# shionhonda/IaGo

Hardware: AMD Instinct MI355X
Metric: self-play games/sec (higher is better)
Workload: dtype f16 MFMA operands (float32 split in 2 / 3 pieces), f32 accumulate; u64 bitboards; f32 / f64 tree statistics

## Files before the change

### iago_amd/csrc/conv_policy_body.hpp

```cpp
#pragma once
#include "abi_common.hpp"

#include <hip/hip_fp16.h>

#include <cstdlib>

#include <atomic>

namespace iago_policy {


typedef _Float16 half8 __attribute__((ext_vector_type(8)));
typedef float float16v __attribute__((ext_vector_type(16)));
typedef float float4v __attribute__((ext_vector_type(4)));
#define IAGO_POLICY_MFMA16(acc, a, b) asm volatile("v_mfma_f32_16x16x32_f16 %0, %1, %2, %0" : "+a"(acc) : "v"(a), "v"(b))
typedef unsigned int u32x4 __attribute__((ext_vector_type(4)));
typedef float f2 __attribute__((ext_vector_type(2)));
typedef _Float16 h2 __attribute__((ext_vector_type(2)));

constexpr int RS = 800;
constexpr int ZB = 1280;
constexpr int BS = 64 * RS + ZB;
constexpr int HEAD_FLOATS = 64;
constexpr int W1_LDS = (64 * 18 + 64) * 4;
constexpr int LDS_BYTES = BS + 1024 + HEAD_FLOATS * 4 + W1_LDS;
constexpr float S1 = 1.0f / 2048.0f, S2 = 1.0f / (2048.0f * 2048.0f);

struct PolicyParams {
    const uint64_t *own, *opp;
    const int64_t *index;
    const int32_t *n_dev;
    int64_t n;
    const float *w1, *b1;
    const uint4 *w_hi[7], *w_mid[7], *w_lo[7];
    const float *bias[7];
    const float *w9, *b10;
    float *probs;
    uint32_t *overflow;
    int layer_lo, layer_hi;
    uint4 *scratch;
    int64_t row_lo, row_hi;
};

__device__ __forceinline__ void split3(const f2 v, h2 &hi, h2 &mid, h2 &lo)
{
    hi = __builtin_convertvector(v, h2);
    const f2 r1 = (v - __builtin_convertvector(hi, f2)) * 2048.0f;
    mid = __builtin_convertvector(r1, h2);
    const f2 r2 = (r1 - __builtin_convertvector(mid, f2)) * 2048.0f;
    lo = __builtin_convertvector(r2, h2);
}

extern __shared__ __align__(16) char policy_lds[];

template <bool SRCH = false>
__device__ __forceinline__ void policy_item(const PolicyParams &P, const int64_t row_id, const uint32_t *pos = nullptr,
                                            float *res = nullptr, const float *w1_staged = nullptr,
                                            const float *head_w = nullptr)
{
    char *const T = policy_lds;
    int tid_ = threadIdx.x;
    if constexpr (SRCH)
        asm volatile("" : "+v"(tid_));
    const int tid = tid_, wv = __builtin_amdgcn_readfirstlane(tid >> 6), lane = tid & 63;
    const int64_t b = P.index ? P.index[row_id] : row_id;

    if (tid < ZB / 16)
        *(uint4 *)(T + 64 * RS + tid * 16) = make_uint4(0, 0, 0, 0);
    bool saturated = false;
    if (P.layer_lo > 0) {
        const uint4 *src = P.scratch + (row_id - P.row_lo) * (64 * RS / 16);
        for (int e = tid; e < 64 * RS / 16; e += 256)
            *(uint4 *)(T + e * 16) = src[e];
    } else {
        const int cell = tid & 63, y = cell >> 3, x = cell & 7;
        const uint64_t bits0 = SRCH ? (((uint64_t)pos[5] << 32) | pos[4]) : P.opp[b];
        const uint64_t bits1 = SRCH ? (((uint64_t)pos[3] << 32) | pos[2]) : P.own[b];
        float in[18];
#pragma unroll
        for (int c = 0; c < 2; c++)
#pragma unroll
            for (int ky = 0; ky < 3; ky++)
#pragma unroll
                for (int kx = 0; kx < 3; kx++) {
                    const int yy = y + ky - 1, xx = x + kx - 1;
                    const bool ok = yy >= 0 && yy < 8 && xx >= 0 && xx < 8;
                    const int a = (yy * 8 + xx) & 63;
                    in[c * 9 + ky * 3 + kx] = (ok && (((c ? bits1 : bits0) >> a) & 1ull)) ? 1.0f : 0.0f;
                }
        const float *w1s = w1_staged;
        if constexpr (!SRCH) {
            float *const st = (float *)(T + BS + 1024 + HEAD_FLOATS * 4);
            for (int e = tid; e < 64 * 18 / 4; e += 256)
                ((float4 *)st)[e] = ((const float4 *)P.w1)[e];
            if (tid < 16)
                ((float4 *)(st + 64 * 18))[tid] = ((const float4 *)P.b1)[tid];
            __syncthreads();
            w1s = st;
        }
#pragma unroll 1
        for (int g2 = 0; g2 < 2; g2++) {
            const int grp = __builtin_amdgcn_readfirstlane(g2 * 4 + wv);
            const int co0 = grp * 8;
            _Float16 p0[8], p1[8], p2[8];
#pragma unroll
            for (int k = 0; k < 8; k += 2) {
                const float *wa = w1s + (co0 + k) * 18, *wb = wa + 18;
                f2 acc = (f2){w1s[64 * 18 + co0 + k], w1s[64 * 18 + co0 + k + 1]};
#pragma unroll
                for (int j = 0; j < 18; j++)
                    acc = __builtin_elementwise_fma((f2){wa[j], wb[j]}, (f2){in[j], in[j]}, acc);
                saturated |= !(acc.x <= 65000.0f) || !(acc.y <= 65000.0f);
                f2 v;
                v.x = fminf(fmaxf(acc.x, 0.0f), 65000.0f);
                v.y = fminf(fmaxf(acc.y, 0.0f), 65000.0f);
                h2 a0, a1, a2;
                split3(v, a0, a1, a2);
                p0[k] = a0.x, p0[k + 1] = a0.y;
                p1[k] = a1.x, p1[k + 1] = a1.y;
                p2[k] = a2.x, p2[k + 1] = a2.y;
            }
            char *dst = T + cell * RS + (grp >> 1) * 32 + (grp & 1) * 16;
            *(uint4 *)dst = *(const uint4 *)p0;
            *(uint4 *)(dst + 256) = *(const uint4 *)p1;
            *(uint4 *)(dst + 512) = *(const uint4 *)p2;
        }
    }
    __syncthreads();

    const int c16 = lane & 15, kq = lane >> 4;
    uint32_t addr[4][9];
#pragma unroll
    for (int q = 0; q < 4; q++)
#pragma unroll
        for (int tap = 0; tap < 9; tap++) {
            const int cell = 16 * q + c16;
            const int yy = (cell >> 3) + tap / 3 - 1, xx = (cell & 7) + tap % 3 - 1;
            const bool ok = yy >= 0 && yy < 8 && xx >= 0 && xx < 8;
            const int lin = (cell + (tap / 3 - 1) * 8 + (tap % 3 - 1)) & 7;
            addr[q][tap] = (uint32_t)((ok ? (yy * 8 + xx) * RS : 64 * RS + 32 * lin) + kq * 16);
        }
    uint32_t wrow[4];
#pragma unroll
    for (int q = 0; q < 4; q++)
        wrow[q] = (uint32_t)((16 * q + c16) * RS);

    for (int L = P.layer_lo; L < P.layer_hi; L++) {
        const int n_pairs = L == 0 ? 2 : 4;
        const char *const wh = (const char *)P.w_hi[L], *const wm = (const char *)P.w_mid[L], *const wl = (const char *)P.w_lo[L];
        const uint32_t a_lane = (uint32_t)(((32 * wv + c16) * 2 + (kq & 1) + (kq >> 1) * (9 * 256)) * 16);
        auto a_load = [&](const char *base, uint32_t step_bytes, int m) -> u32x4 {
            return *(const u32x4 *)(base + step_bytes + a_lane + (uint32_t)m * 512u);
        };
        float4v acc0[2][4], acc0b[2][4], acc1[2][4], acc2[2][4];
#pragma unroll
        for (int m = 0; m < 2; m++)
#pragma unroll
            for (int n = 0; n < 4; n++)
#pragma unroll
                for (int v = 0; v < 4; v++) {
                    acc0[m][n][v] = 0.0f;
                    acc0b[m][n][v] = 0.0f;
                    acc1[m][n][v] = 0.0f;
                    acc2[m][n][v] = 0.0f;
                }
        u32x4 a_hi[3][2], a_mid[3][2], a_lo[3][2];
#pragma unroll
        for (int i = 0; i < 2; i++)
#pragma unroll
            for (int m = 0; m < 2; m++) {
                a_hi[i][m] = a_load(wh, (uint32_t)i * 4096u, m);
                a_mid[i][m] = a_load(wm, (uint32_t)i * 4096u, m);
                a_lo[i][m] = a_load(wl, (uint32_t)i * 4096u, m);
            }
        half8 bh[3], bm[3], bl[3];
        auto b_addr = [&](int tile) -> const char * {
            const int over = tile >= 36 ? 64 : 0, tt = tile % 36;
            return T + addr[tt & 3][tt >> 2] + over;
        };
        {
            const char *p0 = b_addr(0), *p1 = b_addr(1);
            bh[0] = *(const half8 *)p0, bm[0] = *(const half8 *)(p0 + 256), bl[0] = *(const half8 *)(p0 + 512);
            bh[1] = *(const half8 *)p1, bm[1] = *(const half8 *)(p1 + 256), bl[1] = *(const half8 *)(p1 + 512);
        }
        for (int cp = 0; cp < n_pairs; cp++) {
#pragma unroll
            for (int tap = 0; tap < 9; tap++) {
                int cp2 = cp, tp2 = tap + 2;
                if (tp2 >= 9) {
                    tp2 -= 9;
                    cp2 += 1;
                }
                if (cp2 >= n_pairs) {
                    cp2 = n_pairs - 1;
                    tp2 = 8;
                }
                const uint32_t w2 = (uint32_t)(18 * cp2 + tp2) * 4096u;
                half8 ah[2], am[2], al[2];
#pragma unroll
                for (int m = 0; m < 2; m++) {
                    ah[m] = __builtin_bit_cast(half8, a_hi[tap % 3][m]);
                    am[m] = __builtin_bit_cast(half8, a_mid[tap % 3][m]);
                    al[m] = __builtin_bit_cast(half8, a_lo[tap % 3][m]);
                }
#pragma unroll
                for (int q = 0; q < 4; q++) {
                    const int tile = tap * 4 + q, cur = tile % 3, nxt = (tile + 2) % 3;
                    const char *p = b_addr(tile + 2);
                    __builtin_amdgcn_sched_barrier(0);
                    IAGO_POLICY_MFMA16(acc2[0][q], ah[0], bl[cur]);
                    bh[nxt] = *(const half8 *)p;
                    __builtin_amdgcn_sched_barrier(0);
                    IAGO_POLICY_MFMA16(acc2[1][q], ah[1], bl[cur]);
                    bm[nxt] = *(const half8 *)(p + 256);
                    __builtin_amdgcn_sched_barrier(0);
                    IAGO_POLICY_MFMA16(acc1[0][q], ah[0], bm[cur]);
                    bl[nxt] = *(const half8 *)(p + 512);
                    __builtin_amdgcn_sched_barrier(0);
                    IAGO_POLICY_MFMA16(acc1[1][q], ah[1], bm[cur]);
                    if (q == 0)
                        a_hi[(tap + 2) % 3][0] = a_load(wh, w2, 0);
                    else if (q == 1)
                        a_mid[(tap + 2) % 3][0] = a_load(wm, w2, 0);
                    else if (q == 2)
                        a_lo[(tap + 2) % 3][0] = a_load(wl, w2, 0);
                    __builtin_amdgcn_sched_barrier(0);
                    if (tap & 1)
                        IAGO_POLICY_MFMA16(acc0b[0][q], ah[0], bh[cur]);
                    else
                        IAGO_POLICY_MFMA16(acc0[0][q], ah[0], bh[cur]);
                    if (q == 0)
                        a_hi[(tap + 2) % 3][1] = a_load(wh, w2, 1);
                    else if (q == 1)
                        a_mid[(tap + 2) % 3][1] = a_load(wm, w2, 1);
                    else if (q == 2)
                        a_lo[(tap + 2) % 3][1] = a_load(wl, w2, 1);
                    __builtin_amdgcn_sched_barrier(0);
                    if (tap & 1)
                        IAGO_POLICY_MFMA16(acc0b[1][q], ah[1], bh[cur]);
                    else
                        IAGO_POLICY_MFMA16(acc0[1][q], ah[1], bh[cur]);
                    IAGO_POLICY_MFMA16(acc2[0][q], al[0], bh[cur]);
                    IAGO_POLICY_MFMA16(acc2[1][q], al[1], bh[cur]);
                    IAGO_POLICY_MFMA16(acc1[0][q], am[0], bh[cur]);
                    IAGO_POLICY_MFMA16(acc1[1][q], am[1], bh[cur]);
                    IAGO_POLICY_MFMA16(acc2[0][q], am[0], bm[cur]);
                    IAGO_POLICY_MFMA16(acc2[1][q], am[1], bm[cur]);
                    __builtin_amdgcn_sched_barrier(0);
                }
            }
#pragma unroll
            for (int q = 0; q < 4; q++)
#pragma unroll
                for (int tap = 0; tap < 9; tap++)
                    addr[q][tap] += 64u;
        }
#pragma unroll
        for (int q = 0; q < 4; q++)
#pragma unroll
            for (int tap = 0; tap < 9; tap++)
                addr[q][tap] -= 64u * (uint32_t)n_pairs;

        f2 bia[2][2];
#pragma unroll
        for (int m = 0; m < 2; m++) {
            const float4 bq = *(const float4 *)(P.bias[L] + 32 * wv + 16 * m + 4 * kq);
            bia[m][0] = (f2){bq.x, bq.y};
            bia[m][1] = (f2){bq.z, bq.w};
        }
        asm volatile("s_nop 15\n\ts_nop 7" ::: "memory");
        __syncthreads();
        float vmax = 0.0f;
        f2 vsum = (f2){0.0f, 0.0f};
#pragma unroll
        for (int q = 0; q < 4; q++) {
            char *row = T + wrow[q] + (32 * wv + 4 * kq) * 2;
#pragma unroll
            for (int m = 0; m < 2; m++) {
                h2 p0[2], p1[2], p2[2];
#pragma unroll
                for (int t2 = 0; t2 < 2; t2++) {
                    const f2 m0 = (f2){acc0[m][q][2 * t2], acc0[m][q][2 * t2 + 1]} + (f2){acc0b[m][q][2 * t2], acc0b[m][q][2 * t2 + 1]};
                    const f2 m1 = (f2){acc1[m][q][2 * t2], acc1[m][q][2 * t2 + 1]};
                    const f2 m2 = (f2){acc2[m][q][2 * t2], acc2[m][q][2 * t2 + 1]};
                    f2 v = (m2 * S2 + m1 * S1) + m0 + bia[m][t2];
                    vmax = fmaxf(fmaxf(vmax, v.x), v.y);
                    vsum += v;
                    v.x = __builtin_amdgcn_fmed3f(v.x, 0.0f, 65000.0f);
                    v.y = __builtin_amdgcn_fmed3f(v.y, 0.0f, 65000.0f);
                    split3(v, p0[t2], p1[t2], p2[t2]);
                }
                *(uint2 *)(row + 32 * m) = (uint2){__builtin_bit_cast(uint32_t, p0[0]), __builtin_bit_cast(uint32_t, p0[1])};
                *(uint2 *)(row + 32 * m + 256) =
                    (uint2){__builtin_bit_cast(uint32_t, p1[0]), __builtin_bit_cast(uint32_t, p1[1])};
                *(uint2 *)(row + 32 * m + 512) =
                    (uint2){__builtin_bit_cast(uint32_t, p2[0]), __builtin_bit_cast(uint32_t, p2[1])};
            }
        }
        saturated |= !(vmax <= 65000.0f) || !(vsum.x + vsum.y == vsum.x + vsum.y);
        __syncthreads();
    }
    if (P.overflow && saturated)
        *P.overflow = 1u;
    if (P.layer_hi < 7) {
        uint4 *dst = P.scratch + (row_id - P.row_lo) * (64 * RS / 16);
        for (int e = tid; e < 64 * RS / 16; e += 256)
            dst[e] = *(const uint4 *)(T + e * 16);
        return;
    }

    if (wv == 0) {
        const char *row = T + lane * RS;
        float acc = 0.0f;
#pragma unroll 4
        for (int c8 = 0; c8 < 16; c8++) {
            const half8 xh = *(const half8 *)(row + c8 * 16), xm = *(const half8 *)(row + 256 + c8 * 16),
                        xl = *(const half8 *)(row + 512 + c8 * 16);
            const float *w9 = SRCH ? head_w : P.w9;
            const float4 wa = *(const float4 *)(w9 + c8 * 8), wb = *(const float4 *)(w9 + c8 * 8 + 4);
            const float w[8] = {wa.x, wa.y, wa.z, wa.w, wb.x, wb.y, wb.z, wb.w};
#pragma unroll
            for (int e = 0; e < 8; e++) {
                const float xv = ((float)xl[e] * S2 + (float)xm[e] * S1) + (float)xh[e];
                acc = fmaf(w[e], xv, acc);
            }
        }
        const float logit = acc + (SRCH ? head_w[128 + lane] : P.b10[lane]);
        float mx = logit;
#pragma unroll
        for (int o = 32; o > 0; o >>= 1)
            mx = fmaxf(mx, __shfl_xor(mx, o));
        const float e = expf(logit - mx);
        float sum = e;
#pragma unroll
        for (int o = 32; o > 0; o >>= 1)
            sum += __shfl_xor(sum, o);
        if constexpr (SRCH)
            res[lane] = e / sum;
        else
            P.probs[row_id * 64 + lane] = e / sum;
    }
}

inline int policy_params_of(const iago_policy_split3_args *a, PolicyParams &P)
{
    if (!a || a->n < 0)
        return iago_fail(IAGO_ERR_INVALID, "iago_policy_forward_split3: null args or n < 0");
    if (!a->own || !a->opp || !a->w1 || !a->b1 || !a->w9 || !a->b10 || !a->probs)
        return iago_fail(IAGO_ERR_INVALID, "iago_policy_forward_split3: null pointer");
    for (int L = 0; L < 7; L++) {
        if (!a->w_hi[L] || !a->w_mid[L] || !a->w_lo[L] || !a->bias[L] || ((uintptr_t)a->w_hi[L] & 15u) ||
            ((uintptr_t)a->w_mid[L] & 15u) || ((uintptr_t)a->w_lo[L] & 15u) || ((uintptr_t)a->bias[L] & 15u))
            return iago_fail(IAGO_ERR_INVALID, "iago_policy_forward_split3: weights and biases of blocks 2..8 must be "
                                               "non-null and 16-byte aligned");
        P.w_hi[L] = (const uint4 *)a->w_hi[L];
        P.w_mid[L] = (const uint4 *)a->w_mid[L];
        P.w_lo[L] = (const uint4 *)a->w_lo[L];
        P.bias[L] = a->bias[L];
    }
    if (((uintptr_t)a->w9 & 15u) || ((uintptr_t)a->w1 & 15u) || ((uintptr_t)a->b1 & 15u))
        return iago_fail(IAGO_ERR_INVALID, "iago_policy_forward_split3: w1, b1, w9 must be 16-byte aligned");
    P.own = a->own;
    P.opp = a->opp;
    P.index = a->index;
    P.n_dev = a->n_dev;
    P.n = a->n;
    P.w1 = a->w1;
    P.b1 = a->b1;
    P.w9 = a->w9;
    P.b10 = a->b10;
    P.probs = a->probs;
    P.overflow = a->overflow;
    P.layer_lo = 0;
    P.layer_hi = 7;
    P.scratch = nullptr;
    P.row_lo = 0;
    P.row_hi = a->n;
    return IAGO_OK;
}

}
```

### iago_amd/csrc/conv_trunk_body.hpp

```cpp
#pragma once
#include "abi_common.hpp"
#include "rollout_row_body.hpp"

#include <hip/hip_fp16.h>

#include <atomic>
#include <type_traits>

namespace iago_trunk {


typedef _Float16 half8 __attribute__((ext_vector_type(8)));
typedef float float16v __attribute__((ext_vector_type(16)));
typedef float float4v __attribute__((ext_vector_type(4)));
typedef unsigned int u32x4 __attribute__((ext_vector_type(4)));
typedef float f2 __attribute__((ext_vector_type(2)));
typedef _Float16 h2 __attribute__((ext_vector_type(2)));

constexpr int RS = 544;
constexpr int ZB = 1024;
constexpr int BS = 64 * RS + ZB;
constexpr int lds_alloc(int tb) { return tb * BS + 1024; }
constexpr int MAX_LAYERS = 8;

#define IAGO_MFMA16(acc, a, b) asm volatile("v_mfma_f32_16x16x32_f16 %0, %1, %2, %0" : "+a"(acc) : "v"(a), "v"(b))

struct TrunkRParams {
    const uint4 *x_hi, *x_lo;
    uint4 *y_hi, *y_lo;
    const uint4 *w_hi[MAX_LAYERS], *w_lo[MAX_LAYERS];
    const float *bias[MAX_LAYERS];
    int64_t n;
    int32_t cin0, n_layers;
    uint32_t *overflow;
    const float *planes;
    const uint64_t *own, *opp;
    const float *w1, *b1;
    const uint4 *w9_hi, *w9_lo;
    const float *b9, *w10, *w11;
    float *out;
    const int64_t *index;
    const int32_t *n_dev;
    int32_t count_lo, count_hi;
    int32_t layer_lo, layer_hi;
    char *scratch;
};
constexpr int IMG = 64 * RS;

struct Piece {
    const int64_t *index;
    const int32_t *n_dev;
    char *scratch;
    int layer_lo, layer_hi;
    const uint32_t *pos;
    float *res;
    const float *w1s;
    const char *head_w;
};
constexpr int HEAD_W_W9LO = 8192, HEAD_W_W10 = 16384, HEAD_W_W11 = 16384 + 32768, HEAD_W_B9 = HEAD_W_W11 + 512,
              HEAD_W_LDS = HEAD_W_B9 + 16;
__device__ __forceinline__ Piece whole_walk(const TrunkRParams &P)
{
    return Piece{P.index, P.n_dev, P.scratch, P.layer_lo, P.layer_hi, nullptr, nullptr, nullptr, nullptr};
}

constexpr int head_lds(int tb) { return (9 * 64 * tb + 64 * tb + 128 * tb) * 4; }
constexpr int W1_LDS = (64 * 18 + 64) * 4;
constexpr int lds_alloc_fused(int tb) { return lds_alloc(tb) + head_lds(tb) + W1_LDS; }

__device__ __forceinline__ int cell_of_lane(int r)
{
    return r < 4 ? r : r < 12 ? 16 + (r - 4) : r < 16 ? 4 + (r - 12) : r < 20 ? 24 + (r - 16) : r < 28 ? 8 + (r - 20)
                                                                                              : 28 + (r - 28);
}

extern __shared__ __align__(16) char trunk_lds[];

constexpr bool tile_off_board(int tb, int tap, int n)
{
    return tb >= 2 && ((tap < 3 && (n & 7) == 0) || (tap >= 6 && (n & 7) == 7));
}
constexpr int kept_before(int tb, int tap, int n)
{
    int k = 0;
    for (int t = 0; t < 9; t++)
        for (int m = 0; m < 4 * tb; m++) {
            if (t == tap && m == n)
                return k;
            k += !tile_off_board(tb, t, m);
        }
    return k;
}
constexpr int kept_tile(int tb, int k)
{
    for (int t = 0; t < 9; t++)
        for (int m = 0; m < 4 * tb; m++)
            if (!tile_off_board(tb, t, m) && k-- == 0)
                return t * 4 * tb + m;
    return -1;
}
template <int I0, int I1, class F>
__device__ __forceinline__ void static_for(F &&f)
{
    if constexpr (I0 < I1) {
        f(std::integral_constant<int, I0>{});
        static_for<I0 + 1, I1>(f);
    }
}

template <bool FUSED, int TB, bool SRCH = false>
__device__ __forceinline__ void trunk_item(const TrunkRParams &P, const Piece &W, const int64_t b0, const int64_t n_rows)
{
    constexpr int NN = 4 * TB;
    char *const T = trunk_lds;
    int tid_ = threadIdx.x;
    if constexpr (SRCH)
        asm volatile("" : "+v"(tid_));
    const int tid = tid_, wv = __builtin_amdgcn_readfirstlane(tid >> 6), lane = tid & 63, r = lane & 31, h = lane >> 5;

    if (tid < TB * (ZB / 16))
        *(uint4 *)(T + (tid / (ZB / 16)) * BS + 64 * RS + (tid % (ZB / 16)) * 16) = make_uint4(0, 0, 0, 0);
    bool saturated = false;
    constexpr bool PIECES = FUSED && TB <= 2;
    if (PIECES && W.layer_lo > 0) {
        constexpr int PER = (TB * (IMG / 16) + 255) / 256;
        uint4 img[PER];
#pragma unroll
        for (int i = 0; i < PER; i++) {
            const int e = min(tid + i * 256, TB * (IMG / 16) - 1);
            const int board = e / (IMG / 16), off = e - board * (IMG / 16);
            const int64_t row = min(b0 + board, n_rows - 1);
            img[i] = ((const uint4 *)(W.scratch + row * IMG))[off];
        }
#pragma unroll
        for (int i = 0; i < PER; i++) {
            const int e = tid + i * 256;
            const int board = e / (IMG / 16), off = e - board * (IMG / 16);
            if (e < TB * (IMG / 16))
                *(uint4 *)(T + board * BS + off * 16) = img[i];
        }
    } else if constexpr (FUSED) {
        const int cell = tid & 63, y = cell >> 3, x = cell & 7;
        float in[TB][18];
#pragma unroll
        for (int board = 0; board < TB; board++) {
            const int64_t row = min(b0 + board, n_rows - 1);
            const int64_t b = W.index ? W.index[row] : row;
            const float *pl = P.planes + b * 128;
            uint64_t bits0, bits1;
            if constexpr (SRCH) {
                const uint32_t *w = W.pos + 6 * board;
                bits1 = ((uint64_t)w[3] << 32) | w[2];
                bits0 = ((uint64_t)w[5] << 32) | w[4];
            } else {
                bits0 = P.planes ? 0ull : P.opp[b];
                bits1 = P.planes ? 0ull : P.own[b];
            }
#pragma unroll
            for (int c = 0; c < 2; c++)
#pragma unroll
                for (int ky = 0; ky < 3; ky++)
#pragma unroll
                    for (int kx = 0; kx < 3; kx++) {
                        const int yy = y + ky - 1, xx = x + kx - 1;
                        const bool ok = yy >= 0 && yy < 8 && xx >= 0 && xx < 8;
                        const int a = (yy * 8 + xx) & 63;
                        float v;
                        if (P.planes)
                            v = ok ? pl[c * 64 + a] : 0.0f;
                        else
                            v = (ok && (((c ? bits1 : bits0) >> a) & 1ull)) ? 1.0f : 0.0f;
                        in[board][c * 9 + ky * 3 + kx] = v;
                    }
        }
        const float *w1s = W.w1s;
        if constexpr (!SRCH) {
            float *const st = (float *)(T + lds_alloc(TB) + head_lds(TB));
            for (int e = tid; e < 64 * 18 / 4; e += 256)
                ((float4 *)st)[e] = ((const float4 *)P.w1)[e];
            if (tid < 16)
                ((float4 *)(st + 64 * 18))[tid] = ((const float4 *)P.b1)[tid];
            __syncthreads();
            w1s = st;
        }
#pragma unroll 1
        for (int g2 = 0; g2 < 2; g2++) {
            const int grp = __builtin_amdgcn_readfirstlane(g2 * 4 + wv);
            const int co0 = grp * 8;
            _Float16 h8[TB][8], l8[TB][8];
#pragma unroll
            for (int k = 0; k < 8; k++) {
                const float *wk = w1s + (co0 + k) * 18;
                const float bk = w1s[64 * 18 + co0 + k];
                float wreg[18];
#pragma unroll
                for (int j = 0; j < 18; j++)
                    wreg[j] = wk[j];
                float accs[TB];
                if constexpr (TB % 2 == 0) {
#pragma unroll
                    for (int bp = 0; bp < TB; bp += 2) {
                        f2 acc = (f2){bk, bk};
#pragma unroll
                        for (int j = 0; j < 18; j++)
                            acc = __builtin_elementwise_fma((f2){wreg[j], wreg[j]}, (f2){in[bp][j], in[bp + 1][j]}, acc);
                        accs[bp] = acc.x;
                        accs[bp + 1] = acc.y;
                    }
                } else {
#pragma unroll
                    for (int board = 0; board < TB; board++) {
                        float acc = bk;
#pragma unroll
                        for (int j = 0; j < 18; j++)
                            acc = fmaf(wreg[j], in[board][j], acc);
                        accs[board] = acc;
                    }
                }
#pragma unroll
                for (int board = 0; board < TB; board++) {
                    const float acc = accs[board];
                    saturated |= !(acc <= 65000.0f);
                    const float v = fminf(fmaxf(acc, 0.0f), 65000.0f);
                    const _Float16 vh = (_Float16)v;
                    h8[board][k] = vh;
                    l8[board][k] = (_Float16)((v - (float)vh) * 2048.0f);
                }
            }
#pragma unroll
            for (int board = 0; board < TB; board++) {
                char *dst = T + board * BS + cell * RS + (grp >> 1) * 32 + (grp & 1) * 16;
                *(uint4 *)dst = *(const uint4 *)h8[board];
                *(uint4 *)(dst + 256) = *(const uint4 *)l8[board];
            }
        }
    } else {
        const int chunks0 = P.cin0 >> 4;
        const int pieces = TB * chunks0 * 128;
        for (int e = tid; e < pieces; e += 256) {
            const int board = e / (chunks0 * 128), rem = e - board * chunks0 * 128;
            const int chunk = rem >> 7, cell = (rem >> 1) & 63, hp = rem & 1;
            const int64_t b = min(b0 + board, P.n - 1);
            const int64_t src = (b * chunks0 + chunk) * 128 + (rem & 127);
            char *dst = T + board * BS + cell * RS + chunk * 32 + hp * 16;
            *(uint4 *)dst = P.x_hi[src];
            *(uint4 *)(dst + 256) = P.x_lo[src];
        }
    }
    __syncthreads();

    constexpr bool ROWS = TB >= 2;
    static_assert(TB == 1 || TB == 2 || TB == 4, "boards per workgroup");
    const int c16 = lane & 15, kq = lane >> 4;
    constexpr int NADDR = ROWS ? 9 : 36;
    uint32_t addr[NADDR];
    uint32_t sx[2] = {0u, 0u};
    uint32_t wrow[ROWS ? 1 : 4];
    if constexpr (ROWS) {
        const int x = c16 & 7, odd = c16 >> 3;
#pragma unroll
        for (int tap = 0; tap < 9; tap++) {
            const int row = tap < 3 ? 1 : 0;
            const int yy = row + tap / 3 - 1, xx = x + tap % 3 - 1;
            const bool ok = xx >= 0 && xx < 8;
            addr[tap] = (uint32_t)(odd * BS + (ok ? (yy * 8 + xx) * RS : 64 * RS + 32 * (xx & 7)) + kq * 16);
        }
        sx[0] = x > 0 ? 8u * RS : 0u;
        sx[1] = x < 7 ? 8u * RS : 0u;
        wrow[0] = (uint32_t)(odd * BS + x * RS);
    } else {
#pragma unroll
        for (int q = 0; q < 4; q++)
#pragma unroll
            for (int tap = 0; tap < 9; tap++) {
                const int cell = 16 * q + c16;
                const int yy = (cell >> 3) + tap / 3 - 1, xx = (cell & 7) + tap % 3 - 1;
                const bool ok = yy >= 0 && yy < 8 && xx >= 0 && xx < 8;
                const int lin = (cell + (tap / 3 - 1) * 8 + (tap % 3 - 1)) & 7;
                addr[9 * q + tap] = (uint32_t)((ok ? (yy * 8 + xx) * RS : 64 * RS + 32 * lin) + kq * 16);
            }
#pragma unroll
        for (int q = 0; q < 4; q++)
            wrow[q] = (uint32_t)((16 * q + c16) * RS);
    }
    auto b_off = [&](int tap, int n) -> uint32_t {
        if constexpr (ROWS) {
            const int dx = tap % 3 - 1, r = (n & 7) - (tap < 3 ? 1 : 0);
            return addr[tap] + (uint32_t)r * (dx == 0 ? 8u * RS : sx[dx > 0]) + (uint32_t)(n >> 3) * (2u * BS);
        } else {
            return addr[9 * n + tap];
        }
    };

    const int L_lo = PIECES ? W.layer_lo : 0, L_hi = PIECES ? W.layer_hi : P.n_layers;
    for (int L = L_lo; L < L_hi; L++) {
        const int n_pairs = L == 0 ? (P.cin0 >> 5) : 4;
        const char *const wh = (const char *)P.w_hi[L], *const wl = (const char *)P.w_lo[L];
        const uint32_t a_lane = (uint32_t)(((32 * wv + c16) * 2 + (kq & 1) + (kq >> 1) * (9 * 256)) * 16);
        auto a_load = [&](const char *base, uint32_t step_bytes, int m) -> u32x4 {
            return *(const u32x4 *)(base + step_bytes + a_lane + (uint32_t)m * 512u);
        };
        float4v acc_main[2][NN], acc_cross[2][NN];
#pragma unroll
        for (int m = 0; m < 2; m++)
#pragma unroll
            for (int n = 0; n < NN; n++)
#pragma unroll
                for (int v = 0; v < 4; v++) {
                    acc_main[m][n][v] = 0.0f;
                    acc_cross[m][n][v] = 0.0f;
                }

        u32x4 a_hi[3][2], a_lo[3][2];
#pragma unroll
        for (int i = 0; i < 2; i++)
#pragma unroll
            for (int m = 0; m < 2; m++) {
                a_hi[i][m] = a_load(wh, (uint32_t)i * 4096u, m);
                a_lo[i][m] = a_load(wl, (uint32_t)i * 4096u, m);
            }
        constexpr int KEPT = kept_before(TB, 9, 0), NR = KEPT % 4 == 0 ? 4 : 6;
        static_assert(KEPT % NR == 0, "the B ring must line up at every chunk pair");
        half8 bh[NR], bl[NR];
        static_for<0, 3>([&](auto kc) __attribute__((always_inline)) {
            constexpr int tile = kept_tile(TB, decltype(kc)::value);
            const char *p0 = T + b_off(tile / NN, tile % NN);
            bh[decltype(kc)::value] = *(const half8 *)p0;
            bl[decltype(kc)::value] = *(const half8 *)(p0 + 256);
        });
        for (int cp = 0; cp < n_pairs; cp++) {
            static_for<0, KEPT>([&](auto kc) __attribute__((always_inline)) {
                constexpr int k = decltype(kc)::value, tile = kept_tile(TB, k), tap = tile / NN, n = tile % NN;
                constexpr int j = k - kept_before(TB, tap, 0);
                static_assert(kept_before(TB, tap + 1, 0) - kept_before(TB, tap, 0) >= 4, "four A loads per k-step");
                constexpr int kn = k + 3, tile_n = kept_tile(TB, kn % KEPT), cur = k % NR, nxt = kn % NR;
                constexpr uint32_t over = kn >= KEPT ? 64u : 0u;
                int cp2 = cp, tp2 = tap + 2;
                if (tp2 >= 9) {
                    tp2 -= 9;
                    cp2 += 1;
                }
                if (cp2 >= n_pairs) {
                    cp2 = n_pairs - 1;
                    tp2 = 8;
                }
                const uint32_t w2 = (uint32_t)(18 * cp2 + tp2) * 4096u;
                const half8 ah0 = __builtin_bit_cast(half8, a_hi[tap % 3][0]), ah1 = __builtin_bit_cast(half8, a_hi[tap % 3][1]);
                const half8 al0 = __builtin_bit_cast(half8, a_lo[tap % 3][0]), al1 = __builtin_bit_cast(half8, a_lo[tap % 3][1]);
                const char *p = T + b_off(tile_n / NN, tile_n % NN) + over;
                __builtin_amdgcn_sched_barrier(0);
                IAGO_MFMA16(acc_cross[0][n], ah0, bl[cur]);
                bh[nxt] = *(const half8 *)p;
                __builtin_amdgcn_sched_barrier(0);
                IAGO_MFMA16(acc_cross[1][n], ah1, bl[cur]);
                bl[nxt] = *(const half8 *)(p + 256);
                __builtin_amdgcn_sched_barrier(0);
                IAGO_MFMA16(acc_main[0][n], ah0, bh[cur]);
                if constexpr (j == 0)
                    a_hi[(tap + 2) % 3][0] = a_load(wh, w2, 0);
                else if constexpr (j == 1)
                    a_hi[(tap + 2) % 3][1] = a_load(wh, w2, 1);
                else if constexpr (j == 2)
                    a_lo[(tap + 2) % 3][0] = a_load(wl, w2, 0);
                else if constexpr (j == 3)
                    a_lo[(tap + 2) % 3][1] = a_load(wl, w2, 1);
                __builtin_amdgcn_sched_barrier(0);
                IAGO_MFMA16(acc_main[1][n], ah1, bh[cur]);
                IAGO_MFMA16(acc_cross[0][n], al0, bh[cur]);
                IAGO_MFMA16(acc_cross[1][n], al1, bh[cur]);
                __builtin_amdgcn_sched_barrier(0);
            });
#pragma unroll
            for (int i = 0; i < NADDR; i++)
                addr[i] += 64u;
        }
#pragma unroll
        for (int i = 0; i < NADDR; i++)
            addr[i] -= 64u * (uint32_t)n_pairs;

        f2 bia[2][2];
#pragma unroll
        for (int m = 0; m < 2; m++) {
            const float4 bq = *(const float4 *)(P.bias[L] + 32 * wv + 16 * m + 4 * kq);
            bia[m][0] = (f2){bq.x, bq.y};
            bia[m][1] = (f2){bq.z, bq.w};
        }
        asm volatile("s_nop 15\n\ts_nop 7" ::: "memory");
        __syncthreads();
        float vmax = 0.0f;
        f2 vsum = (f2){0.0f, 0.0f};
#pragma unroll
        for (int n = 0; n < NN; n++) {
            char *row = T + (ROWS ? wrow[0] + (n & 7) * (8 * RS) + (n >> 3) * (2 * BS) : wrow[ROWS ? 0 : n]) + (32 * wv + 4 * kq) * 2;
#pragma unroll
            for (int m = 0; m < 2; m++) {
                h2 hi[2], lo[2];
#pragma unroll
                for (int t2 = 0; t2 < 2; t2++) {
                    const f2 mm = (f2){acc_main[m][n][2 * t2], acc_main[m][n][2 * t2 + 1]};
                    const f2 c = (f2){acc_cross[m][n][2 * t2], acc_cross[m][n][2 * t2 + 1]};
                    f2 v = c * (1.0f / 2048.0f) + mm + bia[m][t2];
                    vmax = fmaxf(fmaxf(vmax, v.x), v.y);
                    vsum += v;
                    v.x = __builtin_amdgcn_fmed3f(v.x, 0.0f, 65000.0f);
                    v.y = __builtin_amdgcn_fmed3f(v.y, 0.0f, 65000.0f);
                    hi[t2] = __builtin_convertvector(v, h2);
                    lo[t2] = __builtin_convertvector((v - __builtin_convertvector(hi[t2], f2)) * 2048.0f, h2);
                }
                *(uint2 *)(row + 32 * m) = (uint2){__builtin_bit_cast(uint32_t, hi[0]), __builtin_bit_cast(uint32_t, hi[1])};
                *(uint2 *)(row + 32 * m + 256) =
                    (uint2){__builtin_bit_cast(uint32_t, lo[0]), __builtin_bit_cast(uint32_t, lo[1])};
            }
        }
        saturated |= !(vmax <= 65000.0f) || !(vsum.x + vsum.y == vsum.x + vsum.y);
        __syncthreads();
    }
    if (P.overflow && saturated)
        *P.overflow = 1u;

    if (PIECES && W.layer_hi < P.n_layers) {
        for (int e = tid; e < TB * (IMG / 16); e += 256) {
            const int board = e / (IMG / 16), off = e - board * (IMG / 16);
            if (b0 + board < n_rows)
                ((uint4 *)(W.scratch + (b0 + board) * IMG))[off] = *(const uint4 *)(T + board * BS + off * 16);
        }
        return;
    }
    if constexpr (FUSED) {
        constexpr int NC = 64 * TB;
        float *const Dm = (float *)(T + lds_alloc(TB));
        float *const h9s = Dm + 9 * NC;
        float *const hid = h9s + NC;
        float4 w10row[16];
        if constexpr (!SRCH) {
#pragma unroll
            for (int c = 0; c < 16; c++)
                w10row[c] = ((const float4 *)(P.w10 + (tid & 127) * 64))[c];
        }
        const float w11j = SRCH ? ((const float *)(W.head_w + HEAD_W_W11))[tid & 127] : P.w11[tid & 127];
        const float b9 = SRCH ? *(const float *)(W.head_w + HEAD_W_B9) : P.b9[0];
        const int lane_cell = cell_of_lane(r);
        if (wv < TB) {
            const u32x4 *w9h = (const u32x4 *)P.w9_hi + r * 2 + h;
            const u32x4 *w9l = (const u32x4 *)P.w9_lo + r * 2 + h;
            float16v hm[2], hc[2];
#pragma unroll
            for (int jt = 0; jt < 2; jt++)
#pragma unroll
                for (int v = 0; v < 16; v++) {
                    hm[jt][v] = 0.0f;
                    hc[jt][v] = 0.0f;
                }
            u32x4 w9a[SRCH ? 1 : 8], w9b[SRCH ? 1 : 8];
            if constexpr (!SRCH) {
#pragma unroll
                for (int c = 0; c < 8; c++) {
                    w9a[c] = w9h[c * 64];
                    w9b[c] = w9l[c * 64];
                }
            }
#pragma unroll
            for (int c = 0; c < 8; c++) {
                const half8 ah = SRCH ? *(const half8 *)(W.head_w + (c * 64 + r * 2 + h) * 16)
                                      : __builtin_bit_cast(half8, w9a[SRCH ? 0 : c]);
                const half8 al = SRCH ? *(const half8 *)(W.head_w + HEAD_W_W9LO + (c * 64 + r * 2 + h) * 16)
                                      : __builtin_bit_cast(half8, w9b[SRCH ? 0 : c]);
#pragma unroll
                for (int jt = 0; jt < 2; jt++) {
                    const int jj = 2 * wv + jt;
                    const char *p = T + (jj >> 1) * BS + (32 * (jj & 1) + lane_cell) * RS + h * 16 + c * 32;
                    const half8 bh9 = *(const half8 *)p, bl9 = *(const half8 *)(p + 256);
                    hm[jt] = __builtin_amdgcn_mfma_f32_32x32x16_f16(ah, bh9, hm[jt], 0, 0, 0);
                    hc[jt] = __builtin_amdgcn_mfma_f32_32x32x16_f16(ah, bl9, hc[jt], 0, 0, 0);
                    hc[jt] = __builtin_amdgcn_mfma_f32_32x32x16_f16(al, bh9, hc[jt], 0, 0, 0);
                }
            }
#pragma unroll
            for (int jt = 0; jt < 2; jt++) {
                const int jj = 2 * wv + jt;
                const int base = (jj >> 1) * 64 + 32 * (jj & 1) + lane_cell;
#pragma unroll
                for (int t = 0; t < 4; t++)
                    Dm[(4 * h + t) * NC + base] = hm[jt][t] + hc[jt][t] * (1.0f / 2048.0f);
                if (h == 0)
                    Dm[8 * NC + base] = hm[jt][4] + hc[jt][4] * (1.0f / 2048.0f);
            }
        }
        __syncthreads();
        if constexpr (SRCH) {
#pragma unroll
            for (int c = 0; c < 16; c++)
                w10row[c] = ((const float4 *)(W.head_w + HEAD_W_W10))[c * 128 + (tid & 127)];
        }
        if (tid < NC) {
            const int cell = tid & 63, y = cell >> 3, x = cell & 7;
            float s9 = 0.0f;
#pragma unroll
            for (int tap = 0; tap < 9; tap++) {
                const int yy = y + tap / 3 - 1, xx = x + tap % 3 - 1;
                if (yy >= 0 && yy < 8 && xx >= 0 && xx < 8)
                    s9 += Dm[tap * NC + (tid & ~63) + yy * 8 + xx];
            }
            h9s[tid] = fmaxf(s9 + b9, 0.0f);
        }
        __syncthreads();
        if ((tid >> 7) * 2 < TB) {
            const int j = tid & 127, pb = (tid >> 7) * 2;
            float s0 = 0.0f, s1 = 0.0f;
#pragma unroll
            for (int c = 0; c < 16; c++) {
                const float4 wq = w10row[c];
                const float4 x0 = *(const float4 *)(h9s + pb * 64 + 4 * c);
                const float4 x1 = *(const float4 *)(h9s + (pb + 1 < TB ? pb + 1 : pb) * 64 + 4 * c);
                s0 = fmaf(wq.x, x0.x, s0);
                s0 = fmaf(wq.y, x0.y, s0);
                s0 = fmaf(wq.z, x0.z, s0);
                s0 = fmaf(wq.w, x0.w, s0);
                s1 = fmaf(wq.x, x1.x, s1);
                s1 = fmaf(wq.y, x1.y, s1);
                s1 = fmaf(wq.z, x1.z, s1);
                s1 = fmaf(wq.w, x1.w, s1);
            }
            hid[pb * 128 + j] = s0 * w11j;
            if (pb + 1 < TB)
                hid[(pb + 1) * 128 + j] = s1 * w11j;
        }
        __syncthreads();
        if (tid < TB && b0 + tid < n_rows) {
            float4 hv[32];
#pragma unroll
            for (int j4 = 0; j4 < 32; j4++)
                hv[j4] = *(const float4 *)(hid + tid * 128 + 4 * j4);
            float v = 0.0f;
#pragma unroll
            for (int j4 = 0; j4 < 32; j4++) {
#pragma clang fp reassociate(off)
                v += hv[j4].x;
                v += hv[j4].y;
                v += hv[j4].z;
                v += hv[j4].w;
            }
            const int64_t row = b0 + tid;
            if constexpr (SRCH)
                W.res[tid] = v;
            else
                P.out[W.index ? W.index[row] : row] = v;
        }
        return;
    }
    for (int e = tid; e < TB * 1024; e += 256) {
        const int board = e >> 10, cb = (e >> 7) & 7, cell = (e >> 1) & 63, hp = e & 1;
        const int64_t b = b0 + board;
        if (b < P.n) {
            const char *src = T + board * BS + cell * RS + cb * 32 + hp * 16;
            P.y_hi[b * 1024 + (e & 1023)] = *(const uint4 *)src;
            P.y_lo[b * 1024 + (e & 1023)] = *(const uint4 *)(src + 256);
        }
    }
}

template <bool FUSED, int TB>
__device__ __forceinline__ void trunk_walk(const TrunkRParams &P, const Piece &W, const int64_t bid, const int64_t nb)
{
    int64_t n_rows = P.n;
    if constexpr (FUSED) {
        if (W.n_dev)
            n_rows = min(P.n, (int64_t)*W.n_dev);
        if (n_rows <= P.count_lo || n_rows > P.count_hi)
            return;
    }
    for (int64_t b0 = bid * TB; b0 < n_rows; b0 += nb * TB) {
        trunk_item<FUSED, TB>(P, W, b0, n_rows);
        __syncthreads();
    }
}

inline int value_params_of(const iago_value_split_args *a, TrunkRParams &P)
{
    if (!a || a->n < 0)
        return iago_fail(IAGO_ERR_INVALID, "iago_value_forward_split: null args or n < 0");
    if ((!a->planes && (!a->own || !a->opp)) || !a->w1 || !a->b1 || !a->w9_hi || !a->w9_lo || !a->b9 || !a->w10 ||
        !a->w11 || !a->out)
        return iago_fail(IAGO_ERR_INVALID, "iago_value_forward_split: null pointer");
    for (int L = 0; L < 7; L++) {
        if (!a->w_hi[L] || !a->w_lo[L] || !a->bias[L] || ((uintptr_t)a->w_hi[L] & 15u) || ((uintptr_t)a->w_lo[L] & 15u) ||
            ((uintptr_t)a->bias[L] & 15u))
            return iago_fail(IAGO_ERR_INVALID, "iago_value_forward_split: weights and biases of blocks 2..8 must be "
                                               "non-null and 16-byte aligned");
        P.w_hi[L] = (const uint4 *)a->w_hi[L];
        P.w_lo[L] = (const uint4 *)a->w_lo[L];
        P.bias[L] = a->bias[L];
    }
    P.w_hi[7] = P.w_hi[6];
    P.w_lo[7] = P.w_lo[6];
    P.bias[7] = P.bias[6];
    if (((uintptr_t)a->w9_hi & 15u) || ((uintptr_t)a->w9_lo & 15u) || ((uintptr_t)a->w10 & 15u) || ((uintptr_t)a->w1 & 15u) ||
        ((uintptr_t)a->b1 & 15u))
        return iago_fail(IAGO_ERR_INVALID, "iago_value_forward_split: w1, b1, w9_hi, w9_lo, w10 must be 16-byte aligned");
    P.x_hi = P.x_lo = nullptr;
    P.y_hi = P.y_lo = nullptr;
    P.n = a->n;
    P.cin0 = 64;
    P.n_layers = 7;
    P.overflow = a->overflow;
    P.planes = a->planes;
    P.own = a->own;
    P.opp = a->opp;
    P.w1 = a->w1;
    P.b1 = a->b1;
    P.w9_hi = (const uint4 *)a->w9_hi;
    P.w9_lo = (const uint4 *)a->w9_lo;
    P.b9 = a->b9;
    P.w10 = a->w10;
    P.w11 = a->w11;
    P.out = a->out;
    if (a->index && a->planes)
        return iago_fail(IAGO_ERR_INVALID, "iago_value_forward_split: a gather list needs the boards, not planes");
    P.index = a->index;
    P.n_dev = a->n_dev;
    P.layer_lo = 0;
    P.layer_hi = 7;
    P.scratch = nullptr;
    return IAGO_OK;
}

}
```

Baseline: 2924.

## Prefetch next layer's first weight slices during current layer tail

New measurement: 2929 (median of 6 runs). Within noise of the previous version (+0.2%).

```diff
diff --git a/iago_amd/csrc/conv_policy_body.hpp b/iago_amd/csrc/conv_policy_body.hpp
--- a/iago_amd/csrc/conv_policy_body.hpp
+++ b/iago_amd/csrc/conv_policy_body.hpp
@@ -64,6 +64,25 @@
         asm volatile("" : "+v"(tid_));
     const int tid = tid_, wv = __builtin_amdgcn_readfirstlane(tid >> 6), lane = tid & 63;
     const int64_t b = P.index ? P.index[row_id] : row_id;
+    const int c16 = lane & 15, kq = lane >> 4;
+
+    const uint32_t a_lane = (uint32_t)(((32 * wv + c16) * 2 + (kq & 1) + (kq >> 1) * (9 * 256)) * 16);
+    auto a_load = [&](const char *base, uint32_t step_bytes, int m) -> u32x4 {
+        return *(const u32x4 *)(base + step_bytes + a_lane + (uint32_t)m * 512u);
+    };
+    u32x4 a_hi[3][2], a_mid[3][2], a_lo[3][2];
+    if (P.layer_lo < P.layer_hi) {
+        const char *const wh0 = (const char *)P.w_hi[P.layer_lo], *const wm0 = (const char *)P.w_mid[P.layer_lo],
+                          *const wl0 = (const char *)P.w_lo[P.layer_lo];
+#pragma unroll
+        for (int i = 0; i < 2; i++)
+#pragma unroll
+            for (int m = 0; m < 2; m++) {
+                a_hi[i][m] = a_load(wh0, (uint32_t)i * 4096u, m);
+                a_mid[i][m] = a_load(wm0, (uint32_t)i * 4096u, m);
+                a_lo[i][m] = a_load(wl0, (uint32_t)i * 4096u, m);
+            }
+    }
 
     if (tid < ZB / 16)
         *(uint4 *)(T + 64 * RS + tid * 16) = make_uint4(0, 0, 0, 0);
@@ -128,7 +147,6 @@
     }
     __syncthreads();
 
-    const int c16 = lane & 15, kq = lane >> 4;
     uint32_t addr[4][9];
 #pragma unroll
     for (int q = 0; q < 4; q++)
@@ -148,10 +166,18 @@
     for (int L = P.layer_lo; L < P.layer_hi; L++) {
         const int n_pairs = L == 0 ? 2 : 4;
         const char *const wh = (const char *)P.w_hi[L], *const wm = (const char *)P.w_mid[L], *const wl = (const char *)P.w_lo[L];
-        const uint32_t a_lane = (uint32_t)(((32 * wv + c16) * 2 + (kq & 1) + (kq >> 1) * (9 * 256)) * 16);
-        auto a_load = [&](const char *base, uint32_t step_bytes, int m) -> u32x4 {
-            return *(const u32x4 *)(base + step_bytes + a_lane + (uint32_t)m * 512u);
-        };
+        const bool more = L + 1 < P.layer_hi;
+        const char *const wh_n = more ? (const char *)P.w_hi[L + 1] : wh, *const wm_n = more ? (const char *)P.w_mid[L + 1] : wm,
+                          *const wl_n = more ? (const char *)P.w_lo[L + 1] : wl;
+        const uint32_t last_step = (uint32_t)(18 * (n_pairs - 1) + 8) * 4096u;
+        const uint32_t step_n0 = more ? 0u : last_step, step_n1 = more ? 4096u : last_step;
+        f2 bia[2][2];
+#pragma unroll
+        for (int m = 0; m < 2; m++) {
+            const float4 bq = *(const float4 *)(P.bias[L] + 32 * wv + 16 * m + 4 * kq);
+            bia[m][0] = (f2){bq.x, bq.y};
+            bia[m][1] = (f2){bq.z, bq.w};
+        }
         float4v acc0[2][4], acc0b[2][4], acc1[2][4], acc2[2][4];
 #pragma unroll
         for (int m = 0; m < 2; m++)
@@ -164,15 +190,6 @@
                     acc1[m][n][v] = 0.0f;
                     acc2[m][n][v] = 0.0f;
                 }
-        u32x4 a_hi[3][2], a_mid[3][2], a_lo[3][2];
-#pragma unroll
-        for (int i = 0; i < 2; i++)
-#pragma unroll
-            for (int m = 0; m < 2; m++) {
-                a_hi[i][m] = a_load(wh, (uint32_t)i * 4096u, m);
-                a_mid[i][m] = a_load(wm, (uint32_t)i * 4096u, m);
-                a_lo[i][m] = a_load(wl, (uint32_t)i * 4096u, m);
-            }
         half8 bh[3], bm[3], bl[3];
         auto b_addr = [&](int tile) -> const char * {
             const int over = tile >= 36 ? 64 : 0, tt = tile % 36;
@@ -184,18 +201,14 @@
             bh[1] = *(const half8 *)p1, bm[1] = *(const half8 *)(p1 + 256), bl[1] = *(const half8 *)(p1 + 512);
         }
         for (int cp = 0; cp < n_pairs; cp++) {
+            const bool wrap = cp + 1 >= n_pairs;
+            const char *const wh_w = wrap ? wh_n : wh, *const wm_w = wrap ? wm_n : wm, *const wl_w = wrap ? wl_n : wl;
+            const uint32_t step_w0 = wrap ? step_n0 : (uint32_t)(18 * (cp + 1)) * 4096u;
+            const uint32_t step_w1 = wrap ? step_n1 : (uint32_t)(18 * (cp + 1) + 1) * 4096u;
 #pragma unroll
             for (int tap = 0; tap < 9; tap++) {
-                int cp2 = cp, tp2 = tap + 2;
-                if (tp2 >= 9) {
-                    tp2 -= 9;
-                    cp2 += 1;
-                }
-                if (cp2 >= n_pairs) {
-                    cp2 = n_pairs - 1;
-                    tp2 = 8;
-                }
-                const uint32_t w2 = (uint32_t)(18 * cp2 + tp2) * 4096u;
+                const char *const wh2 = tap < 7 ? wh : wh_w, *const wm2 = tap < 7 ? wm : wm_w, *const wl2 = tap < 7 ? wl : wl_w;
+                const uint32_t w2 = tap < 7 ? (uint32_t)(18 * cp + tap + 2) * 4096u : tap == 7 ? step_w0 : step_w1;
                 half8 ah[2], am[2], al[2];
 #pragma unroll
                 for (int m = 0; m < 2; m++) {
@@ -219,22 +232,22 @@
                     __builtin_amdgcn_sched_barrier(0);
                     IAGO_POLICY_MFMA16(acc1[1][q], ah[1], bm[cur]);
                     if (q == 0)
-                        a_hi[(tap + 2) % 3][0] = a_load(wh, w2, 0);
+                        a_hi[(tap + 2) % 3][0] = a_load(wh2, w2, 0);
                     else if (q == 1)
-                        a_mid[(tap + 2) % 3][0] = a_load(wm, w2, 0);
+                        a_mid[(tap + 2) % 3][0] = a_load(wm2, w2, 0);
                     else if (q == 2)
-                        a_lo[(tap + 2) % 3][0] = a_load(wl, w2, 0);
+                        a_lo[(tap + 2) % 3][0] = a_load(wl2, w2, 0);
                     __builtin_amdgcn_sched_barrier(0);
                     if (tap & 1)
                         IAGO_POLICY_MFMA16(acc0b[0][q], ah[0], bh[cur]);
                     else
                         IAGO_POLICY_MFMA16(acc0[0][q], ah[0], bh[cur]);
                     if (q == 0)
-                        a_hi[(tap + 2) % 3][1] = a_load(wh, w2, 1);
+                        a_hi[(tap + 2) % 3][1] = a_load(wh2, w2, 1);
                     else if (q == 1)
-                        a_mid[(tap + 2) % 3][1] = a_load(wm, w2, 1);
+                        a_mid[(tap + 2) % 3][1] = a_load(wm2, w2, 1);
                     else if (q == 2)
-                        a_lo[(tap + 2) % 3][1] = a_load(wl, w2, 1);
+                        a_lo[(tap + 2) % 3][1] = a_load(wl2, w2, 1);
                     __builtin_amdgcn_sched_barrier(0);
                     if (tap & 1)
                         IAGO_POLICY_MFMA16(acc0b[1][q], ah[1], bh[cur]);
@@ -261,13 +274,6 @@
             for (int tap = 0; tap < 9; tap++)
                 addr[q][tap] -= 64u * (uint32_t)n_pairs;
 
-        f2 bia[2][2];
-#pragma unroll
-        for (int m = 0; m < 2; m++) {
-            const float4 bq = *(const float4 *)(P.bias[L] + 32 * wv + 16 * m + 4 * kq);
-            bia[m][0] = (f2){bq.x, bq.y};
-            bia[m][1] = (f2){bq.z, bq.w};
-        }
         asm volatile("s_nop 15\n\ts_nop 7" ::: "memory");
         __syncthreads();
         float vmax = 0.0f;
diff --git a/iago_amd/csrc/conv_trunk_body.hpp b/iago_amd/csrc/conv_trunk_body.hpp
--- a/iago_amd/csrc/conv_trunk_body.hpp
+++ b/iago_amd/csrc/conv_trunk_body.hpp
@@ -117,11 +117,29 @@
     if constexpr (SRCH)
         asm volatile("" : "+v"(tid_));
     const int tid = tid_, wv = __builtin_amdgcn_readfirstlane(tid >> 6), lane = tid & 63, r = lane & 31, h = lane >> 5;
+    const int c16 = lane & 15, kq = lane >> 4;
+    constexpr bool PIECES = FUSED && TB <= 2;
+    const int L_lo = PIECES ? W.layer_lo : 0, L_hi = PIECES ? W.layer_hi : P.n_layers;
+
+    const uint32_t a_lane = (uint32_t)(((32 * wv + c16) * 2 + (kq & 1) + (kq >> 1) * (9 * 256)) * 16);
+    auto a_load = [&](const char *base, uint32_t step_bytes, int m) -> u32x4 {
+        return *(const u32x4 *)(base + step_bytes + a_lane + (uint32_t)m * 512u);
+    };
+    u32x4 a_hi[3][2], a_lo[3][2];
+    if (L_lo < L_hi) {
+        const char *const wh0 = (const char *)P.w_hi[L_lo], *const wl0 = (const char *)P.w_lo[L_lo];
+#pragma unroll
+        for (int i = 0; i < 2; i++)
+#pragma unroll
+            for (int m = 0; m < 2; m++) {
+                a_hi[i][m] = a_load(wh0, (uint32_t)i * 4096u, m);
+                a_lo[i][m] = a_load(wl0, (uint32_t)i * 4096u, m);
+            }
+    }
 
     if (tid < TB * (ZB / 16))
         *(uint4 *)(T + (tid / (ZB / 16)) * BS + 64 * RS + (tid % (ZB / 16)) * 16) = make_uint4(0, 0, 0, 0);
     bool saturated = false;
-    constexpr bool PIECES = FUSED && TB <= 2;
     if (PIECES && W.layer_lo > 0) {
         constexpr int PER = (TB * (IMG / 16) + 255) / 256;
         uint4 img[PER];
@@ -251,7 +269,6 @@
 
     constexpr bool ROWS = TB >= 2;
     static_assert(TB == 1 || TB == 2 || TB == 4, "boards per workgroup");
-    const int c16 = lane & 15, kq = lane >> 4;
     constexpr int NADDR = ROWS ? 9 : 36;
     uint32_t addr[NADDR];
     uint32_t sx[2] = {0u, 0u};
@@ -292,14 +309,21 @@
         }
     };
 
-    const int L_lo = PIECES ? W.layer_lo : 0, L_hi = PIECES ? W.layer_hi : P.n_layers;
     for (int L = L_lo; L < L_hi; L++) {
         const int n_pairs = L == 0 ? (P.cin0 >> 5) : 4;
+        __builtin_assume(n_pairs >= 1);
         const char *const wh = (const char *)P.w_hi[L], *const wl = (const char *)P.w_lo[L];
-        const uint32_t a_lane = (uint32_t)(((32 * wv + c16) * 2 + (kq & 1) + (kq >> 1) * (9 * 256)) * 16);
-        auto a_load = [&](const char *base, uint32_t step_bytes, int m) -> u32x4 {
-            return *(const u32x4 *)(base + step_bytes + a_lane + (uint32_t)m * 512u);
-        };
+        const bool more = L + 1 < L_hi;
+        const char *const wh_n = more ? (const char *)P.w_hi[L + 1] : wh, *const wl_n = more ? (const char *)P.w_lo[L + 1] : wl;
+        const uint32_t last_step = (uint32_t)(18 * (n_pairs - 1) + 8) * 4096u;
+        const uint32_t step_n0 = more ? 0u : last_step, step_n1 = more ? 4096u : last_step;
+        f2 bia[2][2];
+#pragma unroll
+        for (int m = 0; m < 2; m++) {
+            const float4 bq = *(const float4 *)(P.bias[L] + 32 * wv + 16 * m + 4 * kq);
+            bia[m][0] = (f2){bq.x, bq.y};
+            bia[m][1] = (f2){bq.z, bq.w};
+        }
         float4v acc_main[2][NN], acc_cross[2][NN];
 #pragma unroll
         for (int m = 0; m < 2; m++)
@@ -311,14 +335,6 @@
                     acc_cross[m][n][v] = 0.0f;
                 }
 
-        u32x4 a_hi[3][2], a_lo[3][2];
-#pragma unroll
-        for (int i = 0; i < 2; i++)
-#pragma unroll
-            for (int m = 0; m < 2; m++) {
-                a_hi[i][m] = a_load(wh, (uint32_t)i * 4096u, m);
-                a_lo[i][m] = a_load(wl, (uint32_t)i * 4096u, m);
-            }
         constexpr int KEPT = kept_before(TB, 9, 0), NR = KEPT % 4 == 0 ? 4 : 6;
         static_assert(KEPT % NR == 0, "the B ring must line up at every chunk pair");
         half8 bh[NR], bl[NR];
@@ -329,22 +345,18 @@
             bl[decltype(kc)::value] = *(const half8 *)(p0 + 256);
         });
         for (int cp = 0; cp < n_pairs; cp++) {
+            const bool wrap = cp + 1 >= n_pairs;
+            const char *const wh_w = wrap ? wh_n : wh, *const wl_w = wrap ? wl_n : wl;
+            const uint32_t step_w0 = wrap ? step_n0 : (uint32_t)(18 * (cp + 1)) * 4096u;
+            const uint32_t step_w1 = wrap ? step_n1 : (uint32_t)(18 * (cp + 1) + 1) * 4096u;
             static_for<0, KEPT>([&](auto kc) __attribute__((always_inline)) {
                 constexpr int k = decltype(kc)::value, tile = kept_tile(TB, k), tap = tile / NN, n = tile % NN;
                 constexpr int j = k - kept_before(TB, tap, 0);
                 static_assert(kept_before(TB, tap + 1, 0) - kept_before(TB, tap, 0) >= 4, "four A loads per k-step");
                 constexpr int kn = k + 3, tile_n = kept_tile(TB, kn % KEPT), cur = k % NR, nxt = kn % NR;
                 constexpr uint32_t over = kn >= KEPT ? 64u : 0u;
-                int cp2 = cp, tp2 = tap + 2;
-                if (tp2 >= 9) {
-                    tp2 -= 9;
-                    cp2 += 1;
-                }
-                if (cp2 >= n_pairs) {
-                    cp2 = n_pairs - 1;
-                    tp2 = 8;
-                }
-                const uint32_t w2 = (uint32_t)(18 * cp2 + tp2) * 4096u;
+                const char *const wh2 = tap < 7 ? wh : wh_w, *const wl2 = tap < 7 ? wl : wl_w;
+                const uint32_t w2 = tap < 7 ? (uint32_t)(18 * cp + tap + 2) * 4096u : tap == 7 ? step_w0 : step_w1;
                 const half8 ah0 = __builtin_bit_cast(half8, a_hi[tap % 3][0]), ah1 = __builtin_bit_cast(half8, a_hi[tap % 3][1]);
                 const half8 al0 = __builtin_bit_cast(half8, a_lo[tap % 3][0]), al1 = __builtin_bit_cast(half8, a_lo[tap % 3][1]);
                 const char *p = T + b_off(tile_n / NN, tile_n % NN) + over;
@@ -357,13 +369,13 @@
                 __builtin_amdgcn_sched_barrier(0);
                 IAGO_MFMA16(acc_main[0][n], ah0, bh[cur]);
                 if constexpr (j == 0)
-                    a_hi[(tap + 2) % 3][0] = a_load(wh, w2, 0);
+                    a_hi[(tap + 2) % 3][0] = a_load(wh2, w2, 0);
                 else if constexpr (j == 1)
-                    a_hi[(tap + 2) % 3][1] = a_load(wh, w2, 1);
+                    a_hi[(tap + 2) % 3][1] = a_load(wh2, w2, 1);
                 else if constexpr (j == 2)
-                    a_lo[(tap + 2) % 3][0] = a_load(wl, w2, 0);
+                    a_lo[(tap + 2) % 3][0] = a_load(wl2, w2, 0);
                 else if constexpr (j == 3)
-                    a_lo[(tap + 2) % 3][1] = a_load(wl, w2, 1);
+                    a_lo[(tap + 2) % 3][1] = a_load(wl2, w2, 1);
                 __builtin_amdgcn_sched_barrier(0);
                 IAGO_MFMA16(acc_main[1][n], ah1, bh[cur]);
                 IAGO_MFMA16(acc_cross[0][n], al0, bh[cur]);
@@ -378,13 +390,6 @@
         for (int i = 0; i < NADDR; i++)
             addr[i] -= 64u * (uint32_t)n_pairs;
 
-        f2 bia[2][2];
-#pragma unroll
-        for (int m = 0; m < 2; m++) {
-            const float4 bq = *(const float4 *)(P.bias[L] + 32 * wv + 16 * m + 4 * kq);
-            bia[m][0] = (f2){bq.x, bq.y};
-            bia[m][1] = (f2){bq.z, bq.w};
-        }
         asm volatile("s_nop 15\n\ts_nop 7" ::: "memory");
         __syncthreads();
         float vmax = 0.0f;
```
